# apache/arrow

Measured on AMD Instinct MI355X. Metric: filter_take_mrows_per_s, higher is better.
Workload: dtype int64; 1 GPU; Filter+Take int64[1000000000] + validity (10% null), boolean mask 10% true, FilterOptions::DROP; take indices = the mask's row numbers (monotonic; indices_nonzero: uint64 through CallFunction, GetTakeIndices: uint32 in the mirror), no boundscheck; inputs = splitmix64 streams of SURVEY.md 8(d) (seeds 1,2,3); rows=1000000000, selected_rows=99992053, parallelism=single-gpu

## Files before the change

arrow_amd/_lib.py:

```python
from __future__ import annotations

import ctypes as C
import os

_HERE = os.path.dirname(os.path.abspath(__file__))
LIB_PATH = os.path.join(_HERE, "libarrow_amd.so")

ARX_OK = 0
ARX_OUT_OF_MEMORY = -1
ARX_INVALID = -4
ARX_CAPACITY_ERROR = -6
ARX_INDEX_ERROR = -7
ARX_NOT_IMPLEMENTED = -10
ARX_DEVICE_ERROR = -100

ABI_VERSION = 5

FILTER_DROP, FILTER_EMIT_NULL = 0, 1
SORT_ASCENDING, SORT_DESCENDING = 0, 1
NULLS_AT_START, NULLS_AT_END = 0, 1


class ArrowAmdError(Exception):
    """Base class; subclasses mirror pyarrow.lib.ArrowInvalid & friends."""
# ... 70 lines not shown
_p, _i64, _int, _u64, _u32, _sz = C.c_void_p, C.c_int64, C.c_int, C.c_uint64, C.c_uint32, C.c_size_t
_span = C.POINTER(ArxSpan)
_bspan = C.POINTER(ArxBinarySpan)

SIGNATURES = {
    "arx_last_error": (C.c_char_p, []),
    "arx_abi_version": (_int, []),
    "arx_device_count": (_int, []),
    "arx_set_option": (_int, [C.c_char_p, _i64]),
    "arx_get_option": (_int, [C.c_char_p, C.POINTER(_i64)]),
    "arx_get_counter": (_i64, [C.c_char_p]),
    "arx_filter_workspace_bytes": (_sz, [_i64]),
    "arx_filter_count": (_int, [_span, _int, _p, _sz, C.POINTER(_i64), _p]),
    "arx_filter_count_async": (_int, [_span, _int, _p, _sz, _p]),
    "arx_filter_count_nulls": (_int, [_span, _span, _int, _p, _sz, C.POINTER(_i64), C.POINTER(_i64), _p]),
    "arx_filter_exec": (_int, [_span, _int, _span, _int, _p, _i64, _p, _p, _p]),
    "arx_mask_to_indices": (_int, [_span, _int, _p, _i64, _int, _p, _p, _p]),
    "arx_filter_compact_form": (_int, [_int, _int, _int, _int, _i64, _i64]),
    "arx_take_workspace_bytes": (_sz, []),
    "arx_check_index_bounds": (_int, [_span, _int, _u64, _p, _sz, _p]),
    "arx_take": (_int, [_span, _int, _span, _int, _p, _p, _p, _p]),
    "arx_take_rows": (_int, [_span, _i64, _span, _int, _p, _p, _p, _p]),
    "arx_take_bits": (_int, [_span, _span, _int, _p, _p, _p, _p]),
    "arx_binary_take_workspace_bytes": (_sz, [_i64]),
    "arx_binary_take_offsets": (_int, [_bspan, _span, _int, _p, _sz, _p, _p, _p, C.POINTER(_i64), _p]),
    "arx_binary_take_data": (_int, [_bspan, _i64, _p, _sz, _p, _i64, _p, _p]),
    "arx_large_binary_take_workspace_bytes": (_sz, [_i64]),
    "arx_large_binary_take_offsets": (_int, [_bspan, _span, _int, _p, _sz, _p, _p, _p, C.POINTER(_i64), _p]),
    "arx_large_binary_take_data": (_int, [_bspan, _i64, _p, _sz, _p, _i64, _p, _p]),
    "arx_list_take_data": (_int, [_bspan, _int, _i64, _p, _sz, _p, _i64, _p, _p]),
    "arx_large_list_take_data": (_int, [_bspan, _int, _i64, _p, _sz, _p, _i64, _p, _p]),
    "arx_plain_byte_array_offsets": (_int, [_p, _sz, _i64, C.c_int32, _p]),
# ... 210 lines not shown
```

arrow_amd/csrc/arrow_plugin.cc:

```cpp
#include <arrow/acero/exec_plan.h>
#include <arrow/acero/hash_join_node.h>
#include <arrow/acero/options.h>
#include <arrow/api.h>
#include <arrow/c/abi.h>
#include <arrow/c/bridge.h>
#include <arrow/c/dlpack_abi.h>
#include <arrow/compute/api.h>
#include <arrow/compute/initialize.h>
#include <arrow/compute/kernel.h>
#include <arrow/compute/registry.h>
#include <arrow/device.h>
#include <arrow/util/bit_util.h>
#include <arrow/util/bitmap_builders.h>
#include <arrow/util/bitmap_ops.h>
#include <arrow/acero/util.h>
#include <arrow/acero/query_context.h>

#include <hip/hip_runtime_api.h>
#include <parquet/column_page.h>
#include <parquet/column_reader.h>
#include <parquet/file_reader.h>
#include <parquet/metadata.h>
#include <parquet/schema.h>
#include <parquet/arrow/schema.h>
// ... 539 lines not shown
int64_t arrow_amd_plugin_acero_guard(int what) {
  return what == 1 ? g_guard_takeovers.load() : what == 2 ? g_guard_refusals.load() : (g_acero_guard_installed.load() ? 1 : 0);
}
int arrow_amd_override_acero_factories(int on) {
  const Status st = OverrideAceroFactories(on);
  if (!st.ok()) {
    t_error = st.ToString();
    return -1;
  }
  return 0;
}
void arrow_amd_plugin_set_min_rows(int64_t n) { g_min_rows.store(n); }
void arrow_amd_plugin_set_string_key_hash_bits(int64_t bits) { g_string_key_hash_bits.store(bits < 0 ? 0 : (bits > 64 ? 64 : bits)); }
int64_t arrow_amd_plugin_string_key_hash_collisions(void) { return g_string_key_hash_collisions.load(); }
void arrow_amd_plugin_set_filter_morsel_rows(int64_t n) { g_filter_morsel_rows.store(n); }
void arrow_amd_plugin_set_parquet_device_snappy(int on) { g_parquet_device_snappy.store(on != 0); }
void arrow_amd_plugin_set_parquet_device_levels(int on) { g_parquet_device_levels.store(on != 0); }
void arrow_amd_plugin_set_parquet_pinned_staging(int on) { g_parquet_pinned_staging.store(on != 0); }
void arrow_amd_plugin_set_parquet_read_threads(int n, int64_t min_part_bytes) {
  g_parquet_read_threads.store(n < 1 ? 1 : (n > 16 ? 16 : n));
  g_parquet_read_part_bytes.store(min_part_bytes < 4096 ? 4096 : min_part_bytes);
}
int64_t arrow_amd_plugin_parquet_device_snappy_pages(void) { return g_parquet_device_snappy_pages.load(); }
void arrow_amd_plugin_set_parquet_device_gzip(int on) { g_parquet_device_gzip.store(on != 0); }
int64_t arrow_amd_plugin_parquet_device_gzip_pages(void) { return g_parquet_device_gzip_pages.load(); }
int64_t arrow_amd_plugin_parquet_copied_pages(void) { return g_parquet_copied_pages.load(); }
void arrow_amd_plugin_set_aggregate_stage_nulls(int on) { g_aggregate_stage_nulls.store(on != 0); }
void arrow_amd_plugin_set_aggregate_flush_rows(int64_t rows) { g_aggregate_flush_rows.store(rows < 1 ? 1 : rows); }
int64_t arrow_amd_plugin_aggregate_flushes(void) { return g_aggregate_flushes.load(); }
void arrow_amd_plugin_set_aggregate_direct_rows(int64_t rows) { g_aggregate_direct_rows.store(rows < 1 ? 1 : rows); }
// ... 15 lines not shown
```

arrow_amd/csrc/plugin/common.inc:

```

std::atomic<int64_t> g_gpu_calls{0};
std::atomic<int64_t> g_stock_calls{0};
std::atomic<int64_t> g_min_rows{1 << 16};
std::atomic<int64_t> g_min_rows_streaming{INT64_MAX};
std::atomic<int64_t> g_filter_morsel_rows{[] {
  const char* env = std::getenv("ARROW_AMD_FILTER_MORSEL_ROWS");
  return env != nullptr ? static_cast<int64_t>(std::strtoll(env, nullptr, 10)) : int64_t(1) << 20;
}()};

std::atomic<bool> g_parquet_pinned_staging{true};
std::atomic<bool> g_parquet_device_levels{true};
std::atomic<int> g_parquet_read_threads{4};
std::atomic<int64_t> g_parquet_read_part_bytes{int64_t(1) << 23};
std::atomic<bool> g_parquet_device_snappy{[] {
  const char* env = std::getenv("ARROW_AMD_PARQUET_DEVICE_SNAPPY");
  return env == nullptr || std::strtoll(env, nullptr, 10) != 0;
}()};
std::atomic<int64_t> g_parquet_device_snappy_pages{0};
std::atomic<bool> g_parquet_device_gzip{true};
std::atomic<int64_t> g_parquet_device_gzip_pages{0};
std::atomic<int64_t> g_parquet_copied_pages{0};

std::atomic<int64_t> g_aggregate_flush_rows{[] {
  const char* env = std::getenv("ARROW_AMD_AGGREGATE_FLUSH_ROWS");
// ... 109 lines not shown
      const size_t want = std::max<size_t>(bytes + bytes / 4, 1 << 20);
      HIP_RETURN_NOT_OK(hipMalloc(&s.ptr, want));
      s.size = want;
    }
    *out = s.ptr;
    return Status::OK();
  }

 private:
  struct Slot { void* ptr = nullptr; size_t size = 0; };
  std::vector<Slot> slots_;
  hipStream_t stream_ = nullptr;
};
thread_local DeviceScratch t_scratch;

class PinnedStaging {
 public:
  ~PinnedStaging() {
    if (ptr_) (void)hipHostFree(ptr_);
  }
  Status Reserve(size_t bytes, uint8_t** out) {
    if (size_ < bytes) {
      if (ptr_) HIP_RETURN_NOT_OK(hipHostFree(ptr_));
      ptr_ = nullptr;
      size_ = 0;
      const size_t want = std::max<size_t>(bytes + bytes / 4, size_t(1) << 20);
      HIP_RETURN_NOT_OK(hipHostMalloc(&ptr_, want, hipHostMallocDefault));
      size_ = want;
    }
    *out = static_cast<uint8_t*>(ptr_);
// ... 113 lines not shown
```

arrow_amd/csrc/plugin/selection.inc:

```
StockKernel g_stock_filter;

arrow::Result<std::unique_ptr<cp::KernelState>> FilterInit(cp::KernelContext* ctx,
                                                           const cp::KernelInitArgs& args) {
  auto state = std::make_unique<ShimState<cp::FilterOptions>>();
  if (g_stock_filter.init) {
    ARROW_ASSIGN_OR_RAISE(state->stock, g_stock_filter.init(ctx, args));
  }
  if (args.options != nullptr) {
    state->options = *static_cast<const cp::FilterOptions*>(args.options);
  }
  return state;
}

Status BooleanTakeOnDevice(const ArxSpan& dv, const ArxSpan& di, int tid, hipStream_t st, ArrayData* out_arr) {
  const int64_t m = di.length;
  const int64_t bytes = ((m + 63) / 64) * 8;
  const bool allocate_validity = dv.null_count != 0 || di.null_count != 0;
  out_arr->length = m;
  out_arr->buffers.resize(2);
  out_arr->buffers[0] = nullptr;
  ARROW_ASSIGN_OR_RAISE(out_arr->buffers[1], AllocDevice(bytes));
  void* d_valid = nullptr;
  void* d_counter = nullptr;
  if (allocate_validity) {
// ... 115 lines not shown
      if (allocate_validity) {
        void* cws = nullptr;
        ARROW_RETURN_NOT_OK(t_scratch.Get(kCounter, 64, &cws));
        ARROW_RETURN_NOT_OK(FromArx(arx_bitmap_popcount(d_valid, 0, n, cws, 64, &set_bits, st)));
      } else {
        HIP_RETURN_NOT_OK(hipStreamSynchronize(st));
      }
      out_arr->length = selected;
      out_arr->null_count = allocate_validity ? selected - set_bits : 0;
      static_cast<RocmBuffer*>(out_arr->buffers[1].get())->Shrink(selected * w);
      if (allocate_validity) static_cast<RocmBuffer*>(out_arr->buffers[0].get())->Shrink(((selected + 63) / 64) * 8);
      CountGpu(kFnFilter);
      return Status::OK();
    }
    int64_t out_len = 0, out_nulls = 0;
    if (allocate_validity) {
      ARROW_RETURN_NOT_OK(FromArx(arx_filter_count_nulls(&dv, &dm, null_sel, ws, ws_bytes, &out_len, &out_nulls, st)));
    } else {
      ARROW_RETURN_NOT_OK(FromArx(arx_filter_count(&dm, null_sel, ws, ws_bytes, &out_len, st)));
    }
    out_arr->length = out_len;
    out_arr->buffers.resize(2);
    ARROW_ASSIGN_OR_RAISE(out_arr->buffers[1], AllocDevice(out_len * w));
    out_arr->buffers[0] = nullptr;
    void* d_valid = nullptr;
    if (allocate_validity) {
      ARROW_ASSIGN_OR_RAISE(out_arr->buffers[0], AllocDevice(((out_len + 63) / 64) * 8));
      d_valid = reinterpret_cast<void*>(out_arr->buffers[0]->mutable_address());
    }
    ARROW_RETURN_NOT_OK(FromArx(arx_filter_exec(&dv, w, &dm, null_sel, ws, out_len,
                                                reinterpret_cast<void*>(out_arr->buffers[1]->mutable_address()),
                                                d_valid, st)));
    out_arr->null_count = allocate_validity ? out_nulls : 0;
    HIP_RETURN_NOT_OK(hipStreamSynchronize(st));
    CountGpu(kFnFilter);
// ... 348 lines not shown
```

arrow_amd/csrc/plugin/vector_hash.inc:

```
enum HashVectorKind { kHashUnique = 0, kHashValueCounts, kHashDictEncode };

struct DeviceHashState : public cp::KernelState {
  HashVectorKind kind = kHashUnique;
  std::unique_ptr<cp::KernelState> stock;
  bool used_stock = false, used_device = false;
  bool encode_nulls = false;
  std::shared_ptr<arrow::DataType> type;
  int width = 0;
  std::shared_ptr<Buffer> table_buf, counts_buf;
  void* table = nullptr;
  int64_t max_groups = 0, num_groups = 0, counts_cap = 0;
};

StockKernel g_stock_unique, g_stock_value_counts, g_stock_dict_encode;
cp::VectorKernel::FinalizeFunc g_stock_unique_finalize = nullptr, g_stock_value_counts_finalize = nullptr,
                               g_stock_dict_encode_finalize = nullptr;

template <HashVectorKind KIND>
const StockKernel& StockHashKernel() {
  return KIND == kHashUnique ? g_stock_unique : KIND == kHashValueCounts ? g_stock_value_counts : g_stock_dict_encode;
}

Status HashUniques(DeviceHashState* s, hipStream_t st, std::shared_ptr<Buffer>* values, std::shared_ptr<Buffer>* validity,
                   int64_t* null_count) {
// ... 301 lines not shown
      ARROW_RETURN_NOT_OK(FromArx(arx_compare_numeric(ARX_CMP_NOT_EQUAL, num, base, nullptr, nullptr, &zero, n,
                                                      reinterpret_cast<uint64_t*>(bits->mutable_address()), st)));
    }
    dm.data = reinterpret_cast<const void*>(bits->address());
    dm.offset = 0;
    if (dm.validity != nullptr && dv.offset != 0) {
      ARROW_ASSIGN_OR_RAISE(rebased, AllocDevice(((n + 63) / 64) * 8 + 8));
      ARROW_RETURN_NOT_OK(FromArx(arx_bitmap_copy(dv.validity, dv.offset, n, reinterpret_cast<void*>(rebased->mutable_address()), st)));
      dm.validity = reinterpret_cast<const void*>(rebased->address());
    }
  }
  const size_t ws_bytes = arx_filter_workspace_bytes(n);
  void* ws = nullptr;
  ARROW_RETURN_NOT_OK(t_scratch.Get(kWs, ws_bytes, &ws));
  int64_t cnt = 0;
  if (n > 0) ARROW_RETURN_NOT_OK(FromArx(arx_filter_count(&dm, ARX_FILTER_DROP, ws, ws_bytes, &cnt, st)));
  void* d_idx = nullptr;
  ARROW_RETURN_NOT_OK(t_scratch.Get(kArg2, static_cast<size_t>(cnt) * 4 + 64, &d_idx));
  ARROW_ASSIGN_OR_RAISE(auto out_values, AllocDevice(std::max<int64_t>(cnt, 1) * 8));
  bool direct = false;
  if (cnt > 0) {
    direct = arx_mask_to_indices(&dm, ARX_FILTER_DROP, ws, cnt, 8, reinterpret_cast<void*>(out_values->mutable_address()), nullptr, st) == ARX_OK;
  }
  if (cnt > 0 && !direct) {
    ARROW_RETURN_NOT_OK(FromArx(arx_mask_to_indices(&dm, ARX_FILTER_DROP, ws, cnt, 4, d_idx, nullptr, st)));
    ArxSpan di{nullptr, d_idx, 0, cnt, 0};
    void* flag = nullptr;
    ARROW_RETURN_NOT_OK(t_scratch.Get(kFlag, 64, &flag));
    ARROW_RETURN_NOT_OK(FromArx(arx_cast_numeric(&di, ARX_NUM_UINT32, ARX_NUM_UINT64, 1, 1, flag, 64,
                                                 reinterpret_cast<void*>(out_values->mutable_address()), st)));
  }
  HIP_RETURN_NOT_OK(hipStreamSynchronize(st));
  CountGpu(kFnFilter);
  out->value = ArrayData::Make(arrow::uint64(), cnt, {nullptr, std::move(out_values)}, 0);
  return Status::OK();
}

Status RegisterIndicesNonZero(cp::FunctionRegistry* reg) {
  ARROW_ASSIGN_OR_RAISE(auto fn, reg->GetFunction("indices_nonzero"));
// ... 72 lines not shown
```

arrow_amd/csrc/selection.hip:

```cpp
#include "arx_common.h"

#include <string.h>

#include <algorithm>
#include <type_traits>

namespace arx {

struct FilterWsHeader {
  int64_t total;
  int64_t ntiles;
  int64_t ngroups;
  int64_t length;
  int64_t valid;
  int64_t pad[3];
};
static_assert(sizeof(FilterWsHeader) == 64, "header is one 64-byte line");

struct FilterWsView {
  FilterWsHeader* hdr;
  int64_t* group_excl;
  int64_t* group_total;
  uint32_t* tile_counts;
  int64_t* group_valid;
// ... 18 lines not shown

__device__ __forceinline__ uint64_t emit_word(const Bits& mask, const Bits& mvalid, int64_t w,
                                              bool emit_null, bool invert,
                                              uint64_t* mask_valid_out) {
  uint64_t m = load_word(mask, w);
  const uint64_t mv = load_word(mvalid, w);
  *mask_valid_out = mv;
  if (emit_null || invert) {
    const uint64_t in_range = load_word(Bits{nullptr, 0, mask.length, 0}, w);
    if (invert) m = ~m & in_range;
    if (emit_null) return (m | ~mv) & in_range;
  }
  return m & mv;
}

template <bool VALID>
__global__ __launch_bounds__(kBlock) void count_kernel(Bits mask, Bits mvalid, Bits vvalid, int emit_null,
                                                       int invert, int64_t ntiles,
                                                       uint32_t* tile_counts,
                                                       int64_t* group_total, int64_t* group_valid) {
  __shared__ uint32_t wave_sums[kWavesPerBlock];
  __shared__ uint32_t wave_valid[kWavesPerBlock];
  const int lane = lane_id();
  const int wave = threadIdx.x >> 6;
  const int64_t group = blockIdx.x;
  const int64_t t0 = group * kTilesPerGroup + wave * 16;
  uint32_t mine = 0;
  uint32_t kv = 0;
#pragma unroll 4
  for (int i = 0; i < 16; ++i) {
    const int64_t t = t0 + i;
    uint32_t k = 0;
    if (t < ntiles) {
      uint64_t mv;
      const uint64_t e = emit_word(mask, mvalid, t * 64 + lane, emit_null != 0, invert != 0, &mv);
      k = __popcll(e);
      if constexpr (VALID) kv += __popcll(e & mv & load_word(vvalid, t * 64 + lane));
    }
    const uint32_t s = wave_reduce_sum_u32(k);
    if (lane == i) mine = s;
  }
  if (lane < 16) tile_counts[t0 + lane] = mine;
  const uint32_t wsum = wave_reduce_sum_u32(lane < 16 ? mine : 0u);
  if (lane == 0) wave_sums[wave] = wsum;
  if constexpr (VALID) {
    const uint32_t vsum = wave_reduce_sum_u32(kv);
    if (lane == 0) wave_valid[wave] = vsum;
  }
  __syncthreads();
  if (threadIdx.x == 0) {
    int64_t s = 0, v = 0;
    for (int i = 0; i < kWavesPerBlock; ++i) {
      s += wave_sums[i];
      if constexpr (VALID) v += wave_valid[i];
    }
    group_total[group] = s;
    if constexpr (VALID) group_valid[group] = v;
  }
}

__global__ __launch_bounds__(1024) void scan_kernel(const int64_t* group_total, int64_t ngroups,
                                                    int64_t* group_excl, FilterWsHeader* hdr,
                                                    const int64_t* group_valid = nullptr) {
  __shared__ int64_t wave_tot[16];
  __shared__ int64_t carry_s;
  __shared__ unsigned long long valid_s;
  const int tid = threadIdx.x;
  const int lane = tid & 63;
  const int wave = tid >> 6;
  if (tid == 0) carry_s = 0;
  if (tid == 0) valid_s = 0;
  __syncthreads();
  if (group_valid != nullptr) {
    int64_t mine = 0;
    for (int64_t i = tid; i < ngroups; i += 1024) mine += group_valid[i];
#pragma unroll
    for (int d = 32; d >= 1; d >>= 1) mine += __shfl_xor(mine, d, 64);
    if (lane == 0 && mine != 0) atomicAdd(&valid_s, static_cast<unsigned long long>(mine));
// ... 8 lines not shown
      const int64_t n = __shfl_up(x, d, 64);
      if (lane >= d) x += n;
    }
    if (lane == 63) wave_tot[wave] = x;
    __syncthreads();
    int64_t wave_prefix = 0;
    for (int k = 0; k < wave; ++k) wave_prefix += wave_tot[k];
    const int64_t carry = carry_s;
    if (i < ngroups) group_excl[i] = carry + wave_prefix + x - v;
    __syncthreads();
    if (tid == 1023) carry_s = carry + wave_prefix + x;
    __syncthreads();
  }
  if (tid == 0) {
    hdr->total = carry_s;
    hdr->valid = static_cast<int64_t>(valid_s);
  }
}

struct CompactArgs {
  const uint8_t* values;
  Bits mask;
  Bits mvalid;
  Bits vvalid;
  int64_t length;
  int64_t ntiles;
  const uint32_t* tile_counts;
  const int64_t* group_excl;
  uint8_t* out_data;
  uint64_t* out_validity;
  int emit_null;
  int invert;
  int values_aligned16;
};

constexpr int kFlushBytes = 2048;

template <int RING>
struct __attribute__((aligned(16))) CompactLds {
  uint8_t ring[kWavesPerBlock][RING];
  uint64_t vbits[kWavesPerBlock][72];
};

template <int W>
struct ElemT;
template <> struct ElemT<1> { using type = uint8_t; };
template <> struct ElemT<2> { using type = uint16_t; };
template <> struct ElemT<4> { using type = uint32_t; };
template <> struct ElemT<8> { using type = uint64_t; };
// ... 201 lines not shown
  constexpr int R = 16 / W;
  constexpr int kRowsPerIter = kWave * R;
  constexpr int kIters = kTileRows / kRowsPerIter;
  constexpr int kWordsPerIter = kRowsPerIter / 64;
  constexpr int kBatches = kIters / B;
  constexpr int RING = (B <= 2) ? 4096 : 8192;
  static_assert(kIters % B == 0, "batch must divide the iteration count");
  static_assert(!PIPE || kBatches % 2 == 0, "pipelined form walks the batches in pairs");

  __shared__ CompactLds<RING> lds;

  const int lane = lane_id();
  const int wave = __builtin_amdgcn_readfirstlane(threadIdx.x >> 6);
  const int64_t t = static_cast<int64_t>(blockIdx.x) * kWavesPerBlock + wave;
  if (t >= a.ntiles) return;

  const int64_t w = t * 64 + lane;
  uint64_t mv;
  const uint64_t Ew = emit_word(a.mask, a.mvalid, w, EMIT, a.invert != 0, &mv);
  const uint32_t k = __popcll(Ew);
  const uint32_t incl = wave_inclusive_scan_u32(k);
  const uint32_t p = incl - k;
  const uint32_t total = __shfl(incl, 63, 64);
  if (total == 0) return;

  const int64_t grp = t >> 6;
  const int tin = static_cast<int>(t & 63);
  const uint32_t cprev = lane < tin ? a.tile_counts[grp * kTilesPerGroup + lane] : 0u;
  const int64_t off = a.group_excl[grp] + wave_reduce_sum_u32(cprev);

// ... 142 lines not shown
  uint16_t sel[kWavesPerBlock][kSparseWindow];
  uint64_t vs[kWavesPerBlock][64];
  uint64_t zw[kWavesPerBlock][64];
};

template <int W, bool EMIT, bool IOTA>
__global__ __launch_bounds__(kBlock) void compact_sparse_kernel(CompactArgs a) {
  using E = typename ElemT<W>::type;
  constexpr int U = kSparseU;
  __shared__ SparseLds lds;

  const int lane = lane_id();
  const int wave = __builtin_amdgcn_readfirstlane(threadIdx.x >> 6);
  const int64_t t = static_cast<int64_t>(blockIdx.x) * kWavesPerBlock + wave;
  if (t >= a.ntiles) return;

  const int64_t w = t * 64 + lane;
  uint64_t mv;
  const uint64_t Ew = emit_word(a.mask, a.mvalid, w, EMIT, a.invert != 0, &mv);
  const uint32_t k = __popcll(Ew);
  const uint32_t incl = wave_inclusive_scan_u32(k);
  const uint32_t p = incl - k;
  const int total = static_cast<int>(__shfl(incl, 63, 64));
  if (total == 0) return;

  const int64_t grp = t >> 6;
  const int tin = static_cast<int>(t & 63);
  const uint32_t cprev = lane < tin ? a.tile_counts[grp * kTilesPerGroup + lane] : 0u;
  const int64_t off = a.group_excl[grp] + wave_reduce_sum_u32(cprev);

// ... 456 lines not shown
  if (mask->length > 0 && mask->data == nullptr) {
    set_error("filter mask has no data buffer");
    return ARX_INVALID;
  }
  if (null_selection != ARX_FILTER_DROP && null_selection != ARX_FILTER_EMIT_NULL) {
    set_error("bad null_selection %d", null_selection);
    return ARX_INVALID;
  }
  return ARX_OK;
}

static inline const void* effective_validity(const ArxSpan* s) {
  return (s->null_count != 0) ? s->validity : nullptr;
}

static int launch_count(const ArxSpan* mask, int null_selection, void* ws, size_t ws_bytes,
                        hipStream_t st, int invert = 0, const ArxSpan* values = nullptr) {
  const int rc = check_mask(mask, null_selection);
  if (rc != ARX_OK) return rc;
  const size_t need = arx_filter_workspace_bytes(mask->length);
  if (ws == nullptr || ws_bytes < need) {
    set_error("filter workspace too small: %zu < %zu", ws_bytes, need);
    return ARX_INVALID;
  }
  if ((reinterpret_cast<uint64_t>(ws) & 63) != 0) {
    set_error("filter workspace must be 64-byte aligned");
    return ARX_INVALID;
  }
  FilterWsView v = ws_view(ws, mask->length);
  const int64_t nt = num_tiles(mask->length);
  const int64_t ng = num_groups(mask->length);
  FilterWsHeader h{};
  h.total = 0;
  h.ntiles = nt;
  h.ngroups = ng;
  h.length = mask->length;
  ARX_HIP(hipMemcpyAsync(v.hdr, &h, sizeof(h), hipMemcpyHostToDevice, st));
  if (mask->length == 0) return ARX_OK;
  const Bits mb = make_bits(mask->data, mask->offset, mask->length);
  const Bits mvb = make_bits(effective_validity(mask), mask->offset, mask->length);
  if (values != nullptr) {
    const Bits vvb = make_bits(effective_validity(values), values->offset, mask->length);
    hipLaunchKernelGGL((count_kernel<true>), dim3(static_cast<unsigned>(ng)), dim3(kBlock), 0, st, mb, mvb, vvb,
                       null_selection, invert, nt, v.tile_counts, v.group_total, v.group_valid);
    ARX_CHECK_LAUNCH("count_kernel");
    hipLaunchKernelGGL(scan_kernel, dim3(1), dim3(1024), 0, st, v.group_total, ng, v.group_excl, v.hdr,
                       static_cast<const int64_t*>(v.group_valid));
  } else {
    hipLaunchKernelGGL((count_kernel<false>), dim3(static_cast<unsigned>(ng)), dim3(kBlock), 0, st, mb, mvb, mvb,
                       null_selection, invert, nt, v.tile_counts, v.group_total, static_cast<int64_t*>(nullptr));
    ARX_CHECK_LAUNCH("count_kernel");
    hipLaunchKernelGGL(scan_kernel, dim3(1), dim3(1024), 0, st, v.group_total, ng, v.group_excl, v.hdr,
                       static_cast<const int64_t*>(nullptr));
  }
  ARX_CHECK_LAUNCH("scan_kernel");
  return ARX_OK;
}

static Knob<int> g_filter_batch{4};
static Knob<int> g_filter_pipe{1};
static Knob<int> g_filter_sparse{-1};
static const KnobRow kSelectionKnobs[] = {
    {"filter_batch", g_filter_batch, knob_snap_down<1, 4>},
    {"filter_pipe", g_filter_pipe, knob_bool},
    {"filter_sparse", g_filter_sparse, knob_tri},
};
KnobTable selection_knobs() { return knob_table(kSelectionKnobs); }

// ... 101 lines not shown
}

static int zero_out_validity(void* out_validity, int64_t out_length, hipStream_t st) {
  if (out_validity == nullptr) return ARX_OK;
  if ((reinterpret_cast<uint64_t>(out_validity) & 7) != 0) {
    set_error("out_validity must be 8-byte aligned");
    return ARX_INVALID;
  }
  if (out_length < 0) {
    set_error("out_length (from arx_filter_count) is required when out_validity is given");
    return ARX_INVALID;
  }
  if (out_length > 0) {
    ARX_HIP(hipMemsetAsync(out_validity, 0, static_cast<size_t>(ceil_div(out_length, 64)) * 8, st));
  }
  return ARX_OK;
}

size_t selection_workspace_bytes(int64_t length) { return arx_filter_workspace_bytes(length); }

int selection_bit_positions(const void* bitmap, int64_t bit_offset, int64_t length, bool invert,
                            void* ws, size_t ws_bytes, uint32_t* out, int64_t* out_count_host,
                            hipStream_t st) {
  ArxSpan m{};
  m.validity = nullptr;
  m.data = bitmap;
  m.offset = bit_offset;
  m.length = length;
  m.null_count = 0;
  int rc = launch_count(&m, ARX_FILTER_DROP, ws, ws_bytes, st, invert ? 1 : 0);
// ... 26 lines not shown
using namespace arx;

extern "C" {

size_t arx_filter_workspace_bytes(int64_t length) {
  if (length < 0) length = 0;
  const int64_t ng = num_groups(length);
  return static_cast<size_t>(64 + ng * 16 + ng * kTilesPerGroup * 4 + ng * 8 + 64);
}

int arx_filter_count_async(const ArxSpan* mask, int null_selection, void* ws, size_t ws_bytes,
                           void* stream) {
  return launch_count(mask, null_selection, ws, ws_bytes, as_stream(stream));
}

int arx_filter_count_nulls(const ArxSpan* values, const ArxSpan* mask, int null_selection, void* ws, size_t ws_bytes,
                           int64_t* out_length, int64_t* out_null_count, void* stream) {
  if (out_length == nullptr || out_null_count == nullptr || values == nullptr) {
    set_error("values / out_length / out_null_count is NULL");
    return ARX_INVALID;
  }
  if (mask != nullptr && values->length != mask->length) {
    set_error("filter values and mask differ in length (%lld vs %lld)", static_cast<long long>(values->length),
              static_cast<long long>(mask->length));
    return ARX_INVALID;
  }
  hipStream_t st = as_stream(stream);
  const int rc = launch_count(mask, null_selection, ws, ws_bytes, st, 0, values);
  if (rc != ARX_OK) return rc;
  int64_t hdr[5] = {0, 0, 0, 0, 0};
// ... 8 lines not shown
                     int64_t* out_length, void* stream) {
  if (out_length == nullptr) {
    set_error("out_length is NULL");
    return ARX_INVALID;
  }
  hipStream_t st = as_stream(stream);
  const int rc = launch_count(mask, null_selection, ws, ws_bytes, st);
  if (rc != ARX_OK) return rc;
  int64_t total = 0;
  ARX_HIP(hipMemcpyAsync(&total, ws, sizeof(int64_t), hipMemcpyDeviceToHost, st));
  ARX_HIP(hipStreamSynchronize(st));
  *out_length = total;
  return ARX_OK;
}

int arx_filter_exec(const ArxSpan* values, int byte_width, const ArxSpan* mask, int null_selection,
                    const void* ws, int64_t out_length, void* out_data, void* out_validity,
                    void* stream) {
  int rc = check_mask(mask, null_selection);
  if (rc != ARX_OK) return rc;
  if (values == nullptr || ws == nullptr) {
    set_error("values/ws is NULL");
    return ARX_INVALID;
  }
  if (values->length != mask->length) {
    set_error("Array arguments must all be the same length (values %lld vs filter %lld)",
              static_cast<long long>(values->length), static_cast<long long>(mask->length));
    return ARX_INVALID;
  }
  if (mask->length == 0) return ARX_OK;
  if (values->data == nullptr || out_data == nullptr) {
    set_error("values/out data buffer is NULL");
    return ARX_INVALID;
// ... 5 lines not shown
  a.mask = make_bits(mask->data, mask->offset, mask->length);
  a.mvalid = make_bits(effective_validity(mask), mask->offset, mask->length);
  a.vvalid = make_bits(effective_validity(values), values->offset, values->length);
  a.length = mask->length;
  a.ntiles = num_tiles(mask->length);
  a.tile_counts = v.tile_counts;
  a.group_excl = v.group_excl;
  a.out_data = static_cast<uint8_t*>(out_data);
  a.out_validity = static_cast<uint64_t*>(out_validity);
  a.emit_null = null_selection == ARX_FILTER_EMIT_NULL && a.mvalid.base != nullptr;
  a.values_aligned16 = (reinterpret_cast<uint64_t>(a.values) & 15) == 0;
  if ((reinterpret_cast<uint64_t>(out_data) % byte_width) != 0) {
    set_error("out_data is not aligned to the element width");
    return ARX_INVALID;
  }
  rc = zero_out_validity(out_validity, out_length, st);
  if (rc != ARX_OK) return rc;
  return launch_compact(false, byte_width, a, st, out_length);
}

int arx_expand_by_mask(const void* dense, int byte_width, const ArxSpan* mask, const void* ws, void* out_data,
                       void* stream) {
  int rc = check_mask(mask, ARX_FILTER_DROP);
  if (rc != ARX_OK) return rc;
  if (ws == nullptr) {
    set_error("ws is NULL (run arx_filter_count on the mask first)");
    return ARX_INVALID;
  }
  if (mask->length == 0) return ARX_OK;
  if (out_data == nullptr || (reinterpret_cast<uint64_t>(out_data) % byte_width) != 0 ||
      (dense != nullptr && (reinterpret_cast<uint64_t>(dense) % byte_width) != 0)) {
    set_error("expand: NULL or misaligned buffer");
    return ARX_INVALID;
// ... 12 lines not shown
  hipStream_t st = as_stream(stream);
  switch (byte_width) {
    case 1: hipLaunchKernelGGL((expand_kernel<1>), dim3(grid), dim3(kBlock), 0, st, a); break;
    case 2: hipLaunchKernelGGL((expand_kernel<2>), dim3(grid), dim3(kBlock), 0, st, a); break;
    case 4: hipLaunchKernelGGL((expand_kernel<4>), dim3(grid), dim3(kBlock), 0, st, a); break;
    case 8: hipLaunchKernelGGL((expand_kernel<8>), dim3(grid), dim3(kBlock), 0, st, a); break;
    case 16: hipLaunchKernelGGL((expand_kernel<16>), dim3(grid), dim3(kBlock), 0, st, a); break;
    default:
      set_error("unsupported byte width %d for expand", byte_width);
      return ARX_NOT_IMPLEMENTED;
  }
  ARX_CHECK_LAUNCH("expand_kernel");
  return ARX_OK;
}

int arx_mask_to_indices(const ArxSpan* mask, int null_selection, const void* ws, int64_t out_length,
                        int index_width, void* out_indices, void* out_validity, void* stream) {
  int rc = check_mask(mask, null_selection);
  if (rc != ARX_OK) return rc;
  if (ws == nullptr) {
    set_error("ws is NULL");
    return ARX_INVALID;
  }
  if (index_width != 2 && index_width != 4 && index_width != 8) {
    set_error("index_width must be 2, 4 or 8");
    return ARX_INVALID;
  }
  if (index_width == 8 && (g_filter_sparse == 0 || null_selection == ARX_FILTER_EMIT_NULL)) {
    set_error("index_width 8 is served by the gather form with DROP only");
    return ARX_NOT_IMPLEMENTED;
  }
  if (mask->length > static_cast<int64_t>(UINT32_MAX)) {
// ... 17 lines not shown
  a.mvalid = make_bits(effective_validity(mask), mask->offset, mask->length);
  a.vvalid = make_bits(nullptr, 0, mask->length);
  a.length = mask->length;
  a.ntiles = num_tiles(mask->length);
  a.tile_counts = v.tile_counts;
  a.group_excl = v.group_excl;
  a.out_data = static_cast<uint8_t*>(out_indices);
  a.out_validity = static_cast<uint64_t*>(out_validity);
  a.emit_null = null_selection == ARX_FILTER_EMIT_NULL && a.mvalid.base != nullptr;
  a.values_aligned16 = 1;
  const bool emit = a.emit_null != 0;
  if (emit && out_validity == nullptr) {
    set_error("EMIT_NULL with a nullable mask needs out_validity");
    return ARX_INVALID;
  }
  rc = zero_out_validity(out_validity, out_length, st);
  if (rc != ARX_OK) return rc;
  return launch_compact(true, index_width, a, st);
}

int arx_filter_compact_form(int row_numbers, int byte_width, int values_aligned16, int invert, int64_t length,
                            int64_t out_length) {
  return compact_form(row_numbers != 0, byte_width, values_aligned16 != 0, invert != 0, length, out_length);
}

size_t arx_take_workspace_bytes(void) { return sizeof(BoundsWs); }

int arx_check_index_bounds(const ArxSpan* indices, int index_type, uint64_t upper_limit, void* ws,
                           size_t ws_bytes, void* stream) {
  if (indices == nullptr || ws == nullptr || ws_bytes < sizeof(BoundsWs)) {
    set_error("bad arguments to arx_check_index_bounds");
    return ARX_INVALID;
  }
// ... 337 lines not shown
```

include/arrow_amd.h:

```cpp
#ifndef ARROW_AMD_H_
#define ARROW_AMD_H_

#include <stddef.h>
#include <stdint.h>

#ifdef __cplusplus
extern "C" {
#endif

#define ARX_ABI_VERSION 5

typedef enum ArxStatus {
  ARX_OK = 0,
  ARX_OUT_OF_MEMORY = -1,
  ARX_INVALID = -4,
  ARX_CAPACITY_ERROR = -6,
  ARX_INDEX_ERROR = -7,
  ARX_NOT_IMPLEMENTED = -10,
  ARX_DEVICE_ERROR = -100
} ArxStatus;

enum { ARX_FILTER_DROP = 0, ARX_FILTER_EMIT_NULL = 1 };
enum { ARX_SORT_ASCENDING = 0, ARX_SORT_DESCENDING = 1 };
enum { ARX_NULLS_AT_START = 0, ARX_NULLS_AT_END = 1 };
// ... 18 lines not shown
int arx_get_option(const char* name, int64_t* out_value);
int64_t arx_get_counter(const char* name);


size_t arx_filter_workspace_bytes(int64_t length);

int arx_filter_count(const ArxSpan* mask, int null_selection, void* ws, size_t ws_bytes,
                     int64_t* out_length, void* stream);

int arx_filter_count_nulls(const ArxSpan* values, const ArxSpan* mask, int null_selection, void* ws, size_t ws_bytes,
                           int64_t* out_length, int64_t* out_null_count, void* stream);

int arx_filter_count_async(const ArxSpan* mask, int null_selection, void* ws,
                           size_t ws_bytes, void* stream);

int arx_filter_exec(const ArxSpan* values, int byte_width, const ArxSpan* mask,
                    int null_selection, const void* ws, int64_t out_length, void* out_data,
                    void* out_validity, void* stream);

int arx_mask_to_indices(const ArxSpan* mask, int null_selection, const void* ws,
                        int64_t out_length, int index_width, void* out_indices,
                        void* out_validity, void* stream);

enum { ARX_COMPACT_GATHER = 0, ARX_COMPACT_SWEEP_PIPELINED = 1, ARX_COMPACT_SWEEP_PLAIN = 2, ARX_COMPACT_SWEEP_UNALIGNED = 3 };

int arx_filter_compact_form(int row_numbers, int byte_width, int values_aligned16, int invert,
                            int64_t length, int64_t out_length);

size_t arx_take_workspace_bytes(void);

int arx_check_index_bounds(const ArxSpan* indices, int index_type, uint64_t upper_limit,
                           void* ws, size_t ws_bytes, void* stream);

int arx_take(const ArxSpan* values, int byte_width, const ArxSpan* indices, int index_type,
             void* out_data, void* out_validity, int64_t* valid_count, void* stream);

int arx_take_rows(const ArxSpan* values, int64_t row_bytes, const ArxSpan* indices, int index_type, void* out_data,
// ... 608 lines not shown
```

Before: 313,300 Mrows/s.

## Speculatively size filter output from previous call to skip count sync

Filter and indices_nonzero now reuse the output length of the previous call on the same thread as a speculative capacity. They launch count and a bounded compact back to back without a host round-trip in between, and fall back to the exact path when the real count exceeds that capacity. The count kernel is also rewritten: loads are hoisted into registers, template specialisations handle shifted and absent bitmaps, and tile counts use a packed shuffle reduction. This removes one host synchronisation per call. In exchange it may over-allocate, may need an extra copy or shrink, and wastes a launch when the guess is wrong.

```diff
diff --git a/arrow_amd/_lib.py b/arrow_amd/_lib.py
--- a/arrow_amd/_lib.py
+++ b/arrow_amd/_lib.py
@@ -108,8 +108,11 @@
     "arx_filter_count": (_int, [_span, _int, _p, _sz, C.POINTER(_i64), _p]),
     "arx_filter_count_async": (_int, [_span, _int, _p, _sz, _p]),
     "arx_filter_count_nulls": (_int, [_span, _span, _int, _p, _sz, C.POINTER(_i64), C.POINTER(_i64), _p]),
+    "arx_filter_count_nulls_async": (_int, [_span, _span, _int, _p, _sz, _p]),
     "arx_filter_exec": (_int, [_span, _int, _span, _int, _p, _i64, _p, _p, _p]),
     "arx_mask_to_indices": (_int, [_span, _int, _p, _i64, _int, _p, _p, _p]),
+    "arx_filter_exec_bounded": (_int, [_span, _int, _span, _int, _p, _i64, _p, _p, _p]),
+    "arx_mask_to_indices_bounded": (_int, [_span, _int, _p, _i64, _int, _p, _p, _p]),
     "arx_filter_compact_form": (_int, [_int, _int, _int, _int, _i64, _i64]),
     "arx_take_workspace_bytes": (_sz, []),
     "arx_check_index_bounds": (_int, [_span, _int, _u64, _p, _sz, _p]),
diff --git a/arrow_amd/csrc/arrow_plugin.cc b/arrow_amd/csrc/arrow_plugin.cc
--- a/arrow_amd/csrc/arrow_plugin.cc
+++ b/arrow_amd/csrc/arrow_plugin.cc
@@ -577,6 +577,9 @@
 void arrow_amd_plugin_set_string_key_hash_bits(int64_t bits) { g_string_key_hash_bits.store(bits < 0 ? 0 : (bits > 64 ? 64 : bits)); }
 int64_t arrow_amd_plugin_string_key_hash_collisions(void) { return g_string_key_hash_collisions.load(); }
 void arrow_amd_plugin_set_filter_morsel_rows(int64_t n) { g_filter_morsel_rows.store(n); }
+int64_t arrow_amd_plugin_filter_morsel_rows(void) { return g_filter_morsel_rows.load(); }
+int64_t arrow_amd_plugin_speculative_hits(void) { return g_speculative_hits.load(); }
+int64_t arrow_amd_plugin_speculative_misses(void) { return g_speculative_misses.load(); }
 void arrow_amd_plugin_set_parquet_device_snappy(int on) { g_parquet_device_snappy.store(on != 0); }
 void arrow_amd_plugin_set_parquet_device_levels(int on) { g_parquet_device_levels.store(on != 0); }
 void arrow_amd_plugin_set_parquet_pinned_staging(int on) { g_parquet_pinned_staging.store(on != 0); }
diff --git a/arrow_amd/csrc/plugin/common.inc b/arrow_amd/csrc/plugin/common.inc
--- a/arrow_amd/csrc/plugin/common.inc
+++ b/arrow_amd/csrc/plugin/common.inc
@@ -147,6 +147,22 @@
 };
 thread_local DeviceScratch t_scratch;
 
+enum SpecSite { kSpecFilterW1 = 0, kSpecFilterW2, kSpecFilterW4, kSpecFilterW8, kSpecFilterW16, kSpecFilterW32, kSpecNonZero, kNumSpecSites };
+thread_local int64_t t_spec_length[kNumSpecSites] = {-1, -1, -1, -1, -1, -1, -1};
+std::atomic<int64_t> g_speculative_hits{0};
+std::atomic<int64_t> g_speculative_misses{0};
+inline int SpecFilterSite(int byte_width) {
+  switch (byte_width) {
+    case 1: return kSpecFilterW1;
+    case 2: return kSpecFilterW2;
+    case 4: return kSpecFilterW4;
+    case 8: return kSpecFilterW8;
+    case 16: return kSpecFilterW16;
+    default: return kSpecFilterW32;
+  }
+}
+inline int64_t SpeculativeCapacity(int64_t previous_length) { return previous_length + previous_length / 32 + 64; }
+
 class PinnedStaging {
  public:
   ~PinnedStaging() {
diff --git a/arrow_amd/csrc/plugin/selection.inc b/arrow_amd/csrc/plugin/selection.inc
--- a/arrow_amd/csrc/plugin/selection.inc
+++ b/arrow_amd/csrc/plugin/selection.inc
@@ -153,11 +153,69 @@
       return Status::OK();
     }
     int64_t out_len = 0, out_nulls = 0;
-    if (allocate_validity) {
+    const int site = SpecFilterSite(w);
+    const int64_t previous = t_spec_length[site];
+    if (previous >= 0 && filter.length > 0) {
+      const int64_t capacity = std::min<int64_t>(SpeculativeCapacity(previous), filter.length);
+      if (allocate_validity) {
+        ARROW_RETURN_NOT_OK(FromArx(arx_filter_count_nulls_async(&dv, &dm, null_sel, ws, ws_bytes, st)));
+      } else {
+        ARROW_RETURN_NOT_OK(FromArx(arx_filter_count_async(&dm, null_sel, ws, ws_bytes, st)));
+      }
+      std::shared_ptr<Buffer> data, validity;
+      ARROW_ASSIGN_OR_RAISE(data, AllocDevice(capacity * w));
+      void* d_spec_valid = nullptr;
+      if (allocate_validity) {
+        ARROW_ASSIGN_OR_RAISE(validity, AllocDevice(((capacity + 63) / 64) * 8));
+        d_spec_valid = reinterpret_cast<void*>(validity->mutable_address());
+      }
+      ARROW_RETURN_NOT_OK(FromArx(arx_filter_exec_bounded(&dv, w, &dm, null_sel, ws, capacity,
+                                                          reinterpret_cast<void*>(data->mutable_address()), d_spec_valid, st)));
+      int64_t hdr[5] = {0, 0, 0, 0, 0};
+      HIP_RETURN_NOT_OK(hipMemcpyAsync(hdr, ws, sizeof(hdr), hipMemcpyDeviceToHost, st));
+      HIP_RETURN_NOT_OK(hipStreamSynchronize(st));
+      out_len = hdr[0];
+      out_nulls = allocate_validity ? hdr[0] - hdr[4] : 0;
+      t_spec_length[site] = out_len;
+      if (out_len <= capacity) {
+        g_speculative_hits.fetch_add(1, std::memory_order_relaxed);
+        const int64_t data_bytes = out_len * w, validity_bytes = ((out_len + 63) / 64) * 8;
+        if (out_len * 2 < capacity) {
+          std::shared_ptr<Buffer> exact_data, exact_validity;
+          ARROW_ASSIGN_OR_RAISE(exact_data, AllocDevice(data_bytes));
+          if (data_bytes > 0) {
+            ARROW_RETURN_NOT_OK(FromArx(arx_buffer_copy(reinterpret_cast<const void*>(data->address()),
+                                                        reinterpret_cast<void*>(exact_data->mutable_address()), data_bytes, st)));
+          }
+          if (allocate_validity) {
+            ARROW_ASSIGN_OR_RAISE(exact_validity, AllocDevice(validity_bytes));
+            if (validity_bytes > 0) {
+              ARROW_RETURN_NOT_OK(FromArx(arx_buffer_copy(reinterpret_cast<const void*>(validity->address()),
+                                                          reinterpret_cast<void*>(exact_validity->mutable_address()), validity_bytes, st)));
+            }
+          }
+          HIP_RETURN_NOT_OK(hipStreamSynchronize(st));
+          data = std::move(exact_data);
+          validity = std::move(exact_validity);
+        } else {
+          static_cast<RocmBuffer*>(data.get())->Shrink(data_bytes);
+          if (allocate_validity) static_cast<RocmBuffer*>(validity.get())->Shrink(validity_bytes);
+        }
+        out_arr->length = out_len;
+        out_arr->null_count = out_nulls;
+        out_arr->buffers.resize(2);
+        out_arr->buffers[0] = std::move(validity);
+        out_arr->buffers[1] = std::move(data);
+        CountGpu(kFnFilter);
+        return Status::OK();
+      }
+      g_speculative_misses.fetch_add(1, std::memory_order_relaxed);
+    } else if (allocate_validity) {
       ARROW_RETURN_NOT_OK(FromArx(arx_filter_count_nulls(&dv, &dm, null_sel, ws, ws_bytes, &out_len, &out_nulls, st)));
     } else {
       ARROW_RETURN_NOT_OK(FromArx(arx_filter_count(&dm, null_sel, ws, ws_bytes, &out_len, st)));
     }
+    t_spec_length[site] = out_len;
     out_arr->length = out_len;
     out_arr->buffers.resize(2);
     ARROW_ASSIGN_OR_RAISE(out_arr->buffers[1], AllocDevice(out_len * w));
diff --git a/arrow_amd/csrc/plugin/vector_hash.inc b/arrow_amd/csrc/plugin/vector_hash.inc
--- a/arrow_amd/csrc/plugin/vector_hash.inc
+++ b/arrow_amd/csrc/plugin/vector_hash.inc
@@ -339,15 +339,48 @@
   void* ws = nullptr;
   ARROW_RETURN_NOT_OK(t_scratch.Get(kWs, ws_bytes, &ws));
   int64_t cnt = 0;
-  if (n > 0) ARROW_RETURN_NOT_OK(FromArx(arx_filter_count(&dm, ARX_FILTER_DROP, ws, ws_bytes, &cnt, st)));
-  void* d_idx = nullptr;
-  ARROW_RETURN_NOT_OK(t_scratch.Get(kArg2, static_cast<size_t>(cnt) * 4 + 64, &d_idx));
+  bool counted = false;
+  const int64_t previous = t_spec_length[kSpecNonZero];
+  if (n > 0 && previous >= 0) {
+    const int64_t capacity = std::max<int64_t>(std::min<int64_t>(SpeculativeCapacity(previous), n), 1);
+    ARROW_RETURN_NOT_OK(FromArx(arx_filter_count_async(&dm, ARX_FILTER_DROP, ws, ws_bytes, st)));
+    ARROW_ASSIGN_OR_RAISE(auto spec_values, AllocDevice(capacity * 8));
+    const bool launched = arx_mask_to_indices_bounded(&dm, ARX_FILTER_DROP, ws, capacity, 8,
+                                                      reinterpret_cast<void*>(spec_values->mutable_address()), nullptr, st) == ARX_OK;
+    HIP_RETURN_NOT_OK(hipMemcpyAsync(&cnt, ws, 8, hipMemcpyDeviceToHost, st));
+    HIP_RETURN_NOT_OK(hipStreamSynchronize(st));
+    counted = true;
+    if (launched && cnt <= capacity) {
+      g_speculative_hits.fetch_add(1, std::memory_order_relaxed);
+      const int64_t bytes = std::max<int64_t>(cnt, 1) * 8;
+      if (cnt * 2 < capacity) {
+        ARROW_ASSIGN_OR_RAISE(auto exact, AllocDevice(bytes));
+        if (cnt > 0) {
+          ARROW_RETURN_NOT_OK(FromArx(arx_buffer_copy(reinterpret_cast<const void*>(spec_values->address()),
+                                                      reinterpret_cast<void*>(exact->mutable_address()), cnt * 8, st)));
+          HIP_RETURN_NOT_OK(hipStreamSynchronize(st));
+        }
+        spec_values = std::move(exact);
+      } else {
+        static_cast<RocmBuffer*>(spec_values.get())->Shrink(bytes);
+      }
+      t_spec_length[kSpecNonZero] = cnt;
+      CountGpu(kFnFilter);
+      out->value = ArrayData::Make(arrow::uint64(), cnt, {nullptr, std::move(spec_values)}, 0);
+      return Status::OK();
+    }
+    if (launched) g_speculative_misses.fetch_add(1, std::memory_order_relaxed);
+  }
+  if (n > 0 && !counted) ARROW_RETURN_NOT_OK(FromArx(arx_filter_count(&dm, ARX_FILTER_DROP, ws, ws_bytes, &cnt, st)));
+  t_spec_length[kSpecNonZero] = cnt;
   ARROW_ASSIGN_OR_RAISE(auto out_values, AllocDevice(std::max<int64_t>(cnt, 1) * 8));
   bool direct = false;
   if (cnt > 0) {
     direct = arx_mask_to_indices(&dm, ARX_FILTER_DROP, ws, cnt, 8, reinterpret_cast<void*>(out_values->mutable_address()), nullptr, st) == ARX_OK;
   }
   if (cnt > 0 && !direct) {
+    void* d_idx = nullptr;
+    ARROW_RETURN_NOT_OK(t_scratch.Get(kArg2, static_cast<size_t>(cnt) * 4 + 64, &d_idx));
     ARROW_RETURN_NOT_OK(FromArx(arx_mask_to_indices(&dm, ARX_FILTER_DROP, ws, cnt, 4, d_idx, nullptr, st)));
     ArxSpan di{nullptr, d_idx, 0, cnt, 0};
     void* flag = nullptr;
diff --git a/arrow_amd/csrc/selection.hip b/arrow_amd/csrc/selection.hip
--- a/arrow_amd/csrc/selection.hip
+++ b/arrow_amd/csrc/selection.hip
@@ -56,7 +56,23 @@
   return m & mv;
 }
 
-template <bool VALID>
+template <bool SHIFTED>
+__device__ __forceinline__ uint64_t count_load(const Bits& b, int64_t w) {
+  const int64_t last = b.nphys - 1;
+  uint64_t v = b.base[w < last ? w : last];
+  if constexpr (SHIFTED) {
+    const uint64_t hi = b.base[(w + 1) < last ? (w + 1) : last];
+    v = (v >> b.shift) | ((hi << 1) << (63 - b.shift));
+  }
+  return v;
+}
+
+__device__ __forceinline__ uint64_t in_range_word(int64_t length, int64_t w) {
+  const int64_t remain = length - (w << 6);
+  return remain >= 64 ? ~uint64_t(0) : (remain <= 0 ? uint64_t(0) : ((uint64_t(1) << remain) - 1));
+}
+
+template <bool VALID, bool SHIFTED, bool HAS_MV, bool HAS_VV>
 __global__ __launch_bounds__(kBlock) void count_kernel(Bits mask, Bits mvalid, Bits vvalid, int emit_null,
                                                        int invert, int64_t ntiles,
                                                        uint32_t* tile_counts,
@@ -67,23 +83,53 @@
   const int wave = threadIdx.x >> 6;
   const int64_t group = blockIdx.x;
   const int64_t t0 = group * kTilesPerGroup + wave * 16;
-  uint32_t mine = 0;
+  uint64_t m[16], mv[16], vv[16];
+#pragma unroll
+  for (int i = 0; i < 16; ++i) {
+    const int64_t w = (t0 + i) * 64 + lane;
+    m[i] = count_load<SHIFTED>(mask, w);
+    if constexpr (HAS_MV) mv[i] = count_load<SHIFTED>(mvalid, w);
+    if constexpr (VALID && HAS_VV) vv[i] = count_load<SHIFTED>(vvalid, w);
+  }
+  const uint64_t inv = invert != 0 ? ~uint64_t(0) : 0;
+  const uint64_t en = emit_null != 0 ? ~uint64_t(0) : 0;
+  uint32_t c[16];
   uint32_t kv = 0;
-#pragma unroll 4
+#pragma unroll
   for (int i = 0; i < 16; ++i) {
-    const int64_t t = t0 + i;
-    uint32_t k = 0;
-    if (t < ntiles) {
-      uint64_t mv;
-      const uint64_t e = emit_word(mask, mvalid, t * 64 + lane, emit_null != 0, invert != 0, &mv);
-      k = __popcll(e);
-      if constexpr (VALID) kv += __popcll(e & mv & load_word(vvalid, t * 64 + lane));
-    }
-    const uint32_t s = wave_reduce_sum_u32(k);
-    if (lane == i) mine = s;
-  }
-  if (lane < 16) tile_counts[t0 + lane] = mine;
-  const uint32_t wsum = wave_reduce_sum_u32(lane < 16 ? mine : 0u);
+    const uint64_t in_range = in_range_word(mask.length, (t0 + i) * 64 + lane);
+    const uint64_t mw = (m[i] ^ inv) & in_range;
+    const uint64_t mvw = HAS_MV ? (mv[i] & in_range) : in_range;
+    const uint64_t e = (mw & mvw) | (en & ~mvw & in_range);
+    c[i] = __popcll(e);
+    if constexpr (VALID) kv += __popcll(HAS_VV ? (e & mvw & vv[i]) : (e & mvw));
+  }
+  uint32_t r[8];
+#pragma unroll
+  for (int j = 0; j < 8; ++j) r[j] = c[j] | (c[j + 8] << 16);
+  uint32_t q[4], p[2];
+  {
+    const bool up = (lane & 32) != 0;
+#pragma unroll
+    for (int j = 0; j < 4; ++j) q[j] = (up ? r[j + 4] : r[j]) + __shfl_xor(up ? r[j] : r[j + 4], 32, 64);
+  }
+  {
+    const bool up = (lane & 16) != 0;
+#pragma unroll
+    for (int j = 0; j < 2; ++j) p[j] = (up ? q[j + 2] : q[j]) + __shfl_xor(up ? q[j] : q[j + 2], 16, 64);
+  }
+  uint32_t s;
+  {
+    const bool up = (lane & 8) != 0;
+    s = (up ? p[1] : p[0]) + __shfl_xor(up ? p[0] : p[1], 8, 64);
+  }
+#pragma unroll
+  for (int d = 4; d >= 1; d >>= 1) s += __shfl_xor(s, d, 64);
+  const int j = ((lane >> 5) & 1) * 4 + ((lane >> 4) & 1) * 2 + ((lane >> 3) & 1);
+  const uint32_t lo = s & 0xFFFFu, hi = s >> 16;
+  if ((lane & 7) == 0) tile_counts[t0 + j] = lo;
+  if ((lane & 7) == 1) tile_counts[t0 + j + 8] = hi;
+  const uint32_t wsum = wave_reduce_sum_u32((lane & 7) == 0 ? lo + hi : 0u);
   if (lane == 0) wave_sums[wave] = wsum;
   if constexpr (VALID) {
     const uint32_t vsum = wave_reduce_sum_u32(kv);
@@ -103,7 +149,7 @@
 
 __global__ __launch_bounds__(1024) void scan_kernel(const int64_t* group_total, int64_t ngroups,
                                                     int64_t* group_excl, FilterWsHeader* hdr,
-                                                    const int64_t* group_valid = nullptr) {
+                                                    const int64_t* group_valid, int64_t ntiles, int64_t length) {
   __shared__ int64_t wave_tot[16];
   __shared__ int64_t carry_s;
   __shared__ unsigned long long valid_s;
@@ -142,7 +188,11 @@
   }
   if (tid == 0) {
     hdr->total = carry_s;
+    hdr->ntiles = ntiles;
+    hdr->ngroups = ngroups;
+    hdr->length = length;
     hdr->valid = static_cast<int64_t>(valid_s);
+    hdr->pad[0] = hdr->pad[1] = hdr->pad[2] = 0;
   }
 }
 
@@ -160,7 +210,13 @@
   int emit_null;
   int invert;
   int values_aligned16;
+  int64_t capacity = -1;
+  const FilterWsHeader* hdr = nullptr;
 };
+
+__device__ __forceinline__ bool over_capacity(const CompactArgs& a) {
+  return a.capacity >= 0 && a.hdr->total > a.capacity;
+}
 
 constexpr int kFlushBytes = 2048;
 
@@ -392,6 +448,7 @@
   const int wave = __builtin_amdgcn_readfirstlane(threadIdx.x >> 6);
   const int64_t t = static_cast<int64_t>(blockIdx.x) * kWavesPerBlock + wave;
   if (t >= a.ntiles) return;
+  if (over_capacity(a)) return;
 
   const int64_t w = t * 64 + lane;
   uint64_t mv;
@@ -564,6 +621,7 @@
   const int wave = __builtin_amdgcn_readfirstlane(threadIdx.x >> 6);
   const int64_t t = static_cast<int64_t>(blockIdx.x) * kWavesPerBlock + wave;
   if (t >= a.ntiles) return;
+  if (over_capacity(a)) return;
 
   const int64_t w = t * 64 + lane;
   uint64_t mv;
@@ -1050,6 +1108,36 @@
   return (s->null_count != 0) ? s->validity : nullptr;
 }
 
+template <bool VALID, bool SHIFTED, bool HAS_MV>
+static void launch_count_kernel_v(const Bits& mb, const Bits& mvb, const Bits& vvb, int emit_null, int invert, int64_t nt,
+                                  int64_t ng, uint32_t* tile_counts, int64_t* group_total, int64_t* group_valid,
+                                  hipStream_t st) {
+  const dim3 grid(static_cast<unsigned>(ng)), block(kBlock);
+  if (VALID && vvb.base != nullptr) {
+    hipLaunchKernelGGL((count_kernel<VALID, SHIFTED, HAS_MV, true>), grid, block, 0, st, mb, mvb, vvb, emit_null, invert, nt,
+                       tile_counts, group_total, group_valid);
+  } else {
+    hipLaunchKernelGGL((count_kernel<VALID, SHIFTED, HAS_MV, false>), grid, block, 0, st, mb, mvb, vvb, emit_null, invert, nt,
+                       tile_counts, group_total, group_valid);
+  }
+}
+
+template <bool VALID>
+static void launch_count_kernel(const Bits& mb, const Bits& mvb, const Bits& vvb, int emit_null, int invert, int64_t nt,
+                                int64_t ng, uint32_t* tile_counts, int64_t* group_total, int64_t* group_valid,
+                                hipStream_t st) {
+  const bool has_mv = mvb.base != nullptr;
+  const bool shifted = mb.shift != 0 || (has_mv && mvb.shift != 0) || (VALID && vvb.base != nullptr && vvb.shift != 0);
+#define ARX_COUNT_FORM(S, M) \
+  launch_count_kernel_v<VALID, S, M>(mb, mvb, vvb, emit_null, invert, nt, ng, tile_counts, group_total, group_valid, st)
+  if (shifted) {
+    if (has_mv) ARX_COUNT_FORM(true, true); else ARX_COUNT_FORM(true, false);
+  } else {
+    if (has_mv) ARX_COUNT_FORM(false, true); else ARX_COUNT_FORM(false, false);
+  }
+#undef ARX_COUNT_FORM
+}
+
 static int launch_count(const ArxSpan* mask, int null_selection, void* ws, size_t ws_bytes,
                         hipStream_t st, int invert = 0, const ArxSpan* values = nullptr) {
   const int rc = check_mask(mask, null_selection);
@@ -1066,28 +1154,25 @@
   FilterWsView v = ws_view(ws, mask->length);
   const int64_t nt = num_tiles(mask->length);
   const int64_t ng = num_groups(mask->length);
-  FilterWsHeader h{};
-  h.total = 0;
-  h.ntiles = nt;
-  h.ngroups = ng;
-  h.length = mask->length;
-  ARX_HIP(hipMemcpyAsync(v.hdr, &h, sizeof(h), hipMemcpyHostToDevice, st));
-  if (mask->length == 0) return ARX_OK;
+  if (mask->length == 0) {
+    ARX_HIP(hipMemsetAsync(v.hdr, 0, sizeof(FilterWsHeader), st));
+    return ARX_OK;
+  }
   const Bits mb = make_bits(mask->data, mask->offset, mask->length);
   const Bits mvb = make_bits(effective_validity(mask), mask->offset, mask->length);
+  const int emit_null = null_selection == ARX_FILTER_EMIT_NULL ? 1 : 0;
   if (values != nullptr) {
     const Bits vvb = make_bits(effective_validity(values), values->offset, mask->length);
-    hipLaunchKernelGGL((count_kernel<true>), dim3(static_cast<unsigned>(ng)), dim3(kBlock), 0, st, mb, mvb, vvb,
-                       null_selection, invert, nt, v.tile_counts, v.group_total, v.group_valid);
+    launch_count_kernel<true>(mb, mvb, vvb, emit_null, invert, nt, ng, v.tile_counts, v.group_total, v.group_valid, st);
     ARX_CHECK_LAUNCH("count_kernel");
     hipLaunchKernelGGL(scan_kernel, dim3(1), dim3(1024), 0, st, v.group_total, ng, v.group_excl, v.hdr,
-                       static_cast<const int64_t*>(v.group_valid));
+                       static_cast<const int64_t*>(v.group_valid), nt, mask->length);
   } else {
-    hipLaunchKernelGGL((count_kernel<false>), dim3(static_cast<unsigned>(ng)), dim3(kBlock), 0, st, mb, mvb, mvb,
-                       null_selection, invert, nt, v.tile_counts, v.group_total, static_cast<int64_t*>(nullptr));
+    launch_count_kernel<false>(mb, mvb, make_bits(nullptr, 0, mask->length), emit_null, invert, nt, ng, v.tile_counts,
+                               v.group_total, nullptr, st);
     ARX_CHECK_LAUNCH("count_kernel");
     hipLaunchKernelGGL(scan_kernel, dim3(1), dim3(1024), 0, st, v.group_total, ng, v.group_excl, v.hdr,
-                       static_cast<const int64_t*>(nullptr));
+                       static_cast<const int64_t*>(nullptr), nt, mask->length);
   }
   ARX_CHECK_LAUNCH("scan_kernel");
   return ARX_OK;
@@ -1219,6 +1304,28 @@
   if (out_length > 0) {
     ARX_HIP(hipMemsetAsync(out_validity, 0, static_cast<size_t>(ceil_div(out_length, 64)) * 8, st));
   }
+  return ARX_OK;
+}
+
+__global__ __launch_bounds__(kBlock) void zero_validity_bounded_kernel(uint64_t* __restrict__ out_validity, int64_t nwords,
+                                                                       const FilterWsHeader* hdr, int64_t capacity) {
+  if (hdr->total > capacity) return;
+  const int64_t stride = static_cast<int64_t>(gridDim.x) * kBlock;
+  for (int64_t i = static_cast<int64_t>(blockIdx.x) * kBlock + threadIdx.x; i < nwords; i += stride) out_validity[i] = 0;
+}
+
+static int zero_out_validity_bounded(void* out_validity, int64_t capacity, const FilterWsHeader* hdr, hipStream_t st) {
+  if (out_validity == nullptr) return ARX_OK;
+  if ((reinterpret_cast<uint64_t>(out_validity) & 7) != 0) {
+    set_error("out_validity must be 8-byte aligned");
+    return ARX_INVALID;
+  }
+  const int64_t nwords = ceil_div(capacity, 64);
+  if (nwords == 0) return ARX_OK;
+  const unsigned grid = static_cast<unsigned>(std::min<int64_t>(ceil_div(nwords, kBlock), 2048));
+  hipLaunchKernelGGL(zero_validity_bounded_kernel, dim3(grid), dim3(kBlock), 0, st, static_cast<uint64_t*>(out_validity),
+                     nwords, hdr, capacity);
+  ARX_CHECK_LAUNCH("zero_validity_bounded_kernel");
   return ARX_OK;
 }
 
@@ -1275,6 +1382,20 @@
   return launch_count(mask, null_selection, ws, ws_bytes, as_stream(stream));
 }
 
+int arx_filter_count_nulls_async(const ArxSpan* values, const ArxSpan* mask, int null_selection, void* ws,
+                                 size_t ws_bytes, void* stream) {
+  if (values == nullptr) {
+    set_error("values is NULL");
+    return ARX_INVALID;
+  }
+  if (mask != nullptr && values->length != mask->length) {
+    set_error("filter values and mask differ in length (%lld vs %lld)", static_cast<long long>(values->length),
+              static_cast<long long>(mask->length));
+    return ARX_INVALID;
+  }
+  return launch_count(mask, null_selection, ws, ws_bytes, as_stream(stream), 0, values);
+}
+
 int arx_filter_count_nulls(const ArxSpan* values, const ArxSpan* mask, int null_selection, void* ws, size_t ws_bytes,
                            int64_t* out_length, int64_t* out_null_count, void* stream) {
   if (out_length == nullptr || out_null_count == nullptr || values == nullptr) {
@@ -1313,9 +1434,9 @@
   return ARX_OK;
 }
 
-int arx_filter_exec(const ArxSpan* values, int byte_width, const ArxSpan* mask, int null_selection,
-                    const void* ws, int64_t out_length, void* out_data, void* out_validity,
-                    void* stream) {
+static int filter_exec(const ArxSpan* values, int byte_width, const ArxSpan* mask, int null_selection,
+                       const void* ws, int64_t out_length, int64_t capacity, void* out_data, void* out_validity,
+                       void* stream) {
   int rc = check_mask(mask, null_selection);
   if (rc != ARX_OK) return rc;
   if (values == nullptr || ws == nullptr) {
@@ -1351,9 +1472,32 @@
     set_error("out_data is not aligned to the element width");
     return ARX_INVALID;
   }
-  rc = zero_out_validity(out_validity, out_length, st);
+  if (capacity >= 0) {
+    a.capacity = capacity;
+    a.hdr = v.hdr;
+    rc = zero_out_validity_bounded(out_validity, capacity, v.hdr, st);
+    out_length = capacity;
+  } else {
+    rc = zero_out_validity(out_validity, out_length, st);
+  }
   if (rc != ARX_OK) return rc;
   return launch_compact(false, byte_width, a, st, out_length);
+}
+
+int arx_filter_exec(const ArxSpan* values, int byte_width, const ArxSpan* mask, int null_selection,
+                    const void* ws, int64_t out_length, void* out_data, void* out_validity,
+                    void* stream) {
+  return filter_exec(values, byte_width, mask, null_selection, ws, out_length, -1, out_data, out_validity, stream);
+}
+
+int arx_filter_exec_bounded(const ArxSpan* values, int byte_width, const ArxSpan* mask, int null_selection,
+                            const void* ws, int64_t capacity, void* out_data, void* out_validity,
+                            void* stream) {
+  if (capacity < 0) {
+    set_error("capacity must not be negative");
+    return ARX_INVALID;
+  }
+  return filter_exec(values, byte_width, mask, null_selection, ws, capacity, capacity, out_data, out_validity, stream);
 }
 
 int arx_expand_by_mask(const void* dense, int byte_width, const ArxSpan* mask, const void* ws, void* out_data,
@@ -1396,8 +1540,8 @@
   return ARX_OK;
 }
 
-int arx_mask_to_indices(const ArxSpan* mask, int null_selection, const void* ws, int64_t out_length,
-                        int index_width, void* out_indices, void* out_validity, void* stream) {
+static int mask_to_indices(const ArxSpan* mask, int null_selection, const void* ws, int64_t out_length, int64_t capacity,
+                           int index_width, void* out_indices, void* out_validity, void* stream) {
   int rc = check_mask(mask, null_selection);
   if (rc != ARX_OK) return rc;
   if (ws == nullptr) {
@@ -1445,9 +1589,29 @@
     set_error("EMIT_NULL with a nullable mask needs out_validity");
     return ARX_INVALID;
   }
-  rc = zero_out_validity(out_validity, out_length, st);
+  if (capacity >= 0) {
+    a.capacity = capacity;
+    a.hdr = v.hdr;
+    rc = zero_out_validity_bounded(out_validity, capacity, v.hdr, st);
+  } else {
+    rc = zero_out_validity(out_validity, out_length, st);
+  }
   if (rc != ARX_OK) return rc;
   return launch_compact(true, index_width, a, st);
+}
+
+int arx_mask_to_indices(const ArxSpan* mask, int null_selection, const void* ws, int64_t out_length,
+                        int index_width, void* out_indices, void* out_validity, void* stream) {
+  return mask_to_indices(mask, null_selection, ws, out_length, -1, index_width, out_indices, out_validity, stream);
+}
+
+int arx_mask_to_indices_bounded(const ArxSpan* mask, int null_selection, const void* ws, int64_t capacity,
+                                int index_width, void* out_indices, void* out_validity, void* stream) {
+  if (capacity < 0) {
+    set_error("capacity must not be negative");
+    return ARX_INVALID;
+  }
+  return mask_to_indices(mask, null_selection, ws, capacity, capacity, index_width, out_indices, out_validity, stream);
 }
 
 int arx_filter_compact_form(int row_numbers, int byte_width, int values_aligned16, int invert, int64_t length,
diff --git a/include/arrow_amd.h b/include/arrow_amd.h
--- a/include/arrow_amd.h
+++ b/include/arrow_amd.h
@@ -56,6 +56,9 @@
 int arx_filter_count_async(const ArxSpan* mask, int null_selection, void* ws,
                            size_t ws_bytes, void* stream);
 
+int arx_filter_count_nulls_async(const ArxSpan* values, const ArxSpan* mask, int null_selection, void* ws,
+                                 size_t ws_bytes, void* stream);
+
 int arx_filter_exec(const ArxSpan* values, int byte_width, const ArxSpan* mask,
                     int null_selection, const void* ws, int64_t out_length, void* out_data,
                     void* out_validity, void* stream);
@@ -63,6 +66,13 @@
 int arx_mask_to_indices(const ArxSpan* mask, int null_selection, const void* ws,
                         int64_t out_length, int index_width, void* out_indices,
                         void* out_validity, void* stream);
+
+int arx_filter_exec_bounded(const ArxSpan* values, int byte_width, const ArxSpan* mask,
+                            int null_selection, const void* ws, int64_t capacity, void* out_data,
+                            void* out_validity, void* stream);
+int arx_mask_to_indices_bounded(const ArxSpan* mask, int null_selection, const void* ws,
+                                int64_t capacity, int index_width, void* out_indices,
+                                void* out_validity, void* stream);
 
 enum { ARX_COMPACT_GATHER = 0, ARX_COMPACT_SWEEP_PIPELINED = 1, ARX_COMPACT_SWEEP_PLAIN = 2, ARX_COMPACT_SWEEP_UNALIGNED = 3 };
 
```

After: 318,500 Mrows/s (median of 6 runs). Within noise of the previous version (+1.7%).
